# agnusmaximus/DistributedMNIST

Measured on AMD Instinct MI355X. Metric: images/sec (whole node), MNIST CNN sync-SGD, higher is better.
Workload: dtype bf16; 1 GPU; model=lenet, global_batch=1024, parallelism=dp1, mode=full_sync, mode_requested=full_sync, grad_dtype=fp32

## Files before the change

csrc/bindings.cpp:

```cpp

#include <torch/extension.h>
#include <ATen/hip/HIPContext.h>
#include <hip/hip_runtime.h>

#include <atomic>
#include <map>
#include <tuple>

#include "kernels.h"

namespace {

#define CHECK_BF16(t) TORCH_CHECK((t).scalar_type() == at::kBFloat16, #t " must be bf16")
#define CHECK_F32(t) TORCH_CHECK((t).scalar_type() == at::kFloat, #t " must be fp32")
#define CHECK_CONTIG(t) TORCH_CHECK((t).is_contiguous(), #t " must be contiguous")
#define CHECK_CUDA(t) TORCH_CHECK((t).is_cuda(), #t " must be on GPU")

const unsigned short* bf16_ptr(const torch::Tensor& t) {
  return reinterpret_cast<const unsigned short*>(t.data_ptr());
}
unsigned short* bf16_mut(torch::Tensor& t) {
  return reinterpret_cast<unsigned short*>(t.data_ptr());
}

// ... 693 lines not shown
      d[1].n = 32; d[1].stride = CONV1_DET_PLANE; d[1].P = blocks;
      nd = 2;
    }
    launch_plane_reduce(d, nd, s);
    return;
  }
  if (conv1_mfma_supported(H, W, 1, Cout) && conv1_mfma_enabled() &&
      reinterpret_cast<uintptr_t>(x.data_ptr()) % 8 == 0) {
    launch_conv1_mfma_dw(bf16_ptr(x), bf16_ptr(dyp), am.data_ptr<uint8_t>(),
                         dw_out.data_ptr<float>(),
                         db_out.defined() ? db_out.data_ptr<float>() : nullptr,
                         NB, cur_stream());
    return;
  }
  launch_conv1_dw_pooled(bf16_ptr(x), bf16_ptr(dyp),
                         am.data_ptr<uint8_t>(), dw_out.data_ptr<float>(),
                         db_out.defined() ? db_out.data_ptr<float>() : nullptr,
                         NB, H, W, Cout, cur_stream());
}

torch::Tensor conv_dx(torch::Tensor dact, torch::Tensor w, int64_t Cin) {
  CHECK_BF16(dact); CHECK_CONTIG(dact); CHECK_BF16(w); CHECK_CONTIG(w);
  return conv_dx_step(dact, w, (int)Cin, cur_stream());
}

static void check_pooled(const torch::Tensor& gp, const torch::Tensor& am) {
  CHECK_CUDA(gp); CHECK_BF16(gp); CHECK_CONTIG(gp);
  CHECK_CUDA(am); CHECK_CONTIG(am);
  TORCH_CHECK(am.scalar_type() == at::kByte, "am must be uint8");
  TORCH_CHECK(gp.dim() == 4 && gp.size(1) == 7 && gp.size(2) == 7 &&
                  gp.size(3) == 64,
              "pooled conv2 backward: gp is [NB][7][7][64]");
  TORCH_CHECK(am.numel() == gp.numel(), "am / gp shape mismatch");
  TORCH_CHECK(((uintptr_t)gp.data_ptr() & 15) == 0 &&
                  ((uintptr_t)am.data_ptr() & 7) == 0,
              "pooled conv2 backward: gp 16 B / am 8 B alignment");
}

torch::Tensor conv_dx_pooled(torch::Tensor gp, torch::Tensor am,
                             torch::Tensor w, int64_t Cin, int64_t force_db) {
  check_pooled(gp, am);
  CHECK_BF16(w); CHECK_CONTIG(w);
  TORCH_CHECK(Cin == 32 && w.numel() == 25 * 32 * 64,
              "conv_dx_pooled: LeNet conv2 shapes only");
  TORCH_CHECK(force_db >= 0 && force_db <= 2, "force_db is 0, 1 or 2");
  int NB = gp.size(0);
  auto dx = torch::empty({NB, 14, 14, 32}, gp.options());
  if (NB > 0)
    launch_conv_dx_slab_pooled(bf16_ptr(gp), am.data_ptr<uint8_t>(),
                               bf16_ptr(w), bf16_mut(dx), NB, (int)force_db,
                               cur_stream());
  return dx;
}

void conv_dw_pooled_into(torch::Tensor x, torch::Tensor gp, torch::Tensor am,
                         torch::Tensor dw_out) {
  check_pooled(gp, am);
  CHECK_CUDA(x); CHECK_BF16(x); CHECK_CONTIG(x);
  CHECK_F32(dw_out); CHECK_CONTIG(dw_out);
  TORCH_CHECK(x.dim() == 4 && x.size(0) == gp.size(0) && x.size(1) == 14 &&
                  x.size(2) == 14 && x.size(3) == 32,
              "conv_dw_pooled_into: x is [NB][14][14][32]");
  TORCH_CHECK(dw_out.numel() == 25 * 32 * 64, "conv_dw_pooled_into: dw size");
  TORCH_CHECK(((uintptr_t)x.data_ptr() & 15) == 0, "x 16 B alignment");
  if (det_on()) {
    int NB = x.size(0);
    if (NB <= 0) return;
    auto s = cur_stream();
    int groups = conv2_dw_groups(NB);
    float* planes = det_region(DET_CONV2_DW, x, CONV2_DET_PLANE, groups, s,
                               "conv_dw_pooled_into", "raise DMNIST_DW2_G");
    launch_conv2_dw_slab_pooled_det(bf16_ptr(x), bf16_ptr(gp),
                                    am.data_ptr<uint8_t>(), planes, NB, s);
    reduce_planes(planes, dw_out.data_ptr<float>(), CONV2_DET_PLANE,
                  CONV2_DET_PLANE, groups, s);
    return;
  }
  launch_conv2_dw_slab_pooled(bf16_ptr(x), bf16_ptr(gp),
                              am.data_ptr<uint8_t>(),
                              dw_out.data_ptr<float>(), (int)x.size(0),
                              cur_stream());
}

std::vector<torch::Tensor> softmax_xent_fwd(torch::Tensor logits,
                                            torch::Tensor labels,
                                            c10::optional<torch::Tensor> db_out,
                                            double inv_n) {
  CHECK_CUDA(logits); CHECK_BF16(logits); CHECK_CONTIG(logits);
  TORCH_CHECK(labels.scalar_type() == at::kLong, "labels must be int64");
  CHECK_CONTIG(labels);
  int B = logits.size(0), C = logits.size(1);
  TORCH_CHECK(C <= 16, "softmax_xent kernel supports C<=16");
  TORCH_CHECK(B <= 256 * SOFTMAX_MAX_BLOCKS, "softmax_xent: batch too large");
  auto dl = torch::empty_like(logits);
  auto out = torch::empty({2}, logits.options().dtype(at::kFloat));
  static auto* ws = new WorkspaceSlots(64);
  float* part = device_workspace(
      *ws, logits, 2 * SOFTMAX_MAX_BLOCKS + 1, at::kFloat, cur_stream(),
      "softmax_xent",
      "softmax_xent_fwd: first call on a device allocates its "
      "workspace and must run outside graph capture").data_ptr<float>();
  unsigned* ticket = reinterpret_cast<unsigned*>(part + 2 * SOFTMAX_MAX_BLOCKS);
  float* dbp = nullptr;
  if (db_out.has_value() && db_out->defined())
    dbp = db_out->data_ptr<float>();
  if (det_on() && dbp && B > 0) {
    auto s = cur_stream();
    int blocks = softmax_xent_blocks(B);
    float* planes = det_region(DET_SOFTMAX_DB, logits, C, blocks, s,
                               "softmax_xent_fwd", "lower the batch size");
    launch_softmax_xent_det(bf16_ptr(logits), labels.data_ptr<long>(),
                            bf16_mut(dl), out.data_ptr<float>(), B, C, planes,
                            (float)inv_n, part, ticket, s);
    reduce_planes(planes, dbp, C, C, blocks, s);
  } else {
    launch_softmax_xent(bf16_ptr(logits), labels.data_ptr<long>(),
                        bf16_mut(dl), out.data_ptr<float>(), B, C, dbp,
                        (float)inv_n, part, ticket, cur_stream());
  }
  auto loss = out.select(0, 0);
  auto correct = out.select(0, 1);
  return {loss, correct, dl};
}

static float* ema_ptr(const c10::optional<torch::Tensor>& ema,
                      const torch::Tensor& master, double ema_decay) {
  if (!ema.has_value() || !ema->defined()) return nullptr;
  CHECK_CUDA((*ema)); CHECK_F32((*ema)); CHECK_CONTIG((*ema));
  TORCH_CHECK(ema->numel() >= master.numel(),
              "sgd_step: ema is shorter than master");
  TORCH_CHECK(reinterpret_cast<uintptr_t>(ema->data_ptr()) % 16 == 0,
              "sgd_step: ema must be 16-byte aligned");
  TORCH_CHECK(ema_decay >= 0.0 && ema_decay < 1.0,
              "sgd_step: ema_decay must lie in [0, 1)");
  return ema->data_ptr<float>();
}

static float* momentum_ptr(const c10::optional<torch::Tensor>& momentum) {
  if (!momentum.has_value() || !momentum->defined()) return nullptr;
  CHECK_F32((*momentum)); CHECK_CONTIG((*momentum));
  return momentum->data_ptr<float>();
}

void sgd_step(torch::Tensor master, torch::Tensor grad, torch::Tensor shadow,
              bool has_shadow, double lr, double scale, double dc_keep,
              int64_t seed, int64_t offset,
              c10::optional<torch::Tensor> momentum, double mu,
              c10::optional<torch::Tensor> ema, double ema_decay) {
  CHECK_CUDA(master); CHECK_F32(master); CHECK_CONTIG(master);
  CHECK_F32(grad); CHECK_CONTIG(grad);
  float* mom = momentum_ptr(momentum);
  float* emap = ema_ptr(ema, master, ema_decay);
  launch_sgd_step(master.data_ptr<float>(), grad.data_ptr<float>(),
                  has_shadow ? bf16_mut(shadow) : nullptr,
                  has_shadow ? 1 : 0, master.numel(),
                  (float)(lr * scale), (float)dc_keep, (uint64_t)seed,
                  (uint64_t)offset, mom, (float)mu, emap, (float)ema_decay,
                  cur_stream());
}

void sgd_step_dev(torch::Tensor master, torch::Tensor grad,
                  torch::Tensor shadow, bool has_shadow,
                  torch::Tensor lr_scale_dev, double dc_keep, int64_t seed,
                  torch::Tensor offset_dev,
                  c10::optional<torch::Tensor> momentum, double mu,
                  bool zero_grad, c10::optional<torch::Tensor> ema,
                  double ema_decay) {
  CHECK_CUDA(master); CHECK_F32(master); CHECK_CONTIG(master);
  CHECK_F32(grad); CHECK_CONTIG(grad);
  CHECK_F32(lr_scale_dev);
  float* mom = momentum_ptr(momentum);
  launch_sgd_step_dev(master.data_ptr<float>(), grad.data_ptr<float>(),
                      has_shadow ? bf16_mut(shadow) : nullptr,
                      has_shadow ? 1 : 0, master.numel(),
                      lr_scale_dev.data_ptr<float>(), (float)dc_keep,
                      (uint64_t)seed, offset_dev.data_ptr<long>(),
                      mom, (float)mu, zero_grad ? 1 : 0,
                      ema_ptr(ema, master, ema_decay), (float)ema_decay,
                      cur_stream());
}

void ema_publish(torch::Tensor ema, torch::Tensor shadow,
                 std::vector<int64_t> offsets, std::vector<int64_t> rows,
                 std::vector<int64_t> cols, std::vector<torch::Tensor> dsts) {
  CHECK_CUDA(ema); CHECK_F32(ema); CHECK_CONTIG(ema);
  CHECK_CUDA(shadow); CHECK_BF16(shadow); CHECK_CONTIG(shadow);
  TORCH_CHECK(shadow.numel() == ema.numel(), "ema_publish: shadow size");
  TORCH_CHECK(reinterpret_cast<uintptr_t>(ema.data_ptr()) % 16 == 0 &&
              reinterpret_cast<uintptr_t>(shadow.data_ptr()) % 8 == 0,
              "ema_publish: ema must be 16-byte and shadow 8-byte aligned");
  size_t nt = dsts.size();
  TORCH_CHECK(nt <= 4 && offsets.size() == nt && rows.size() == nt &&
              cols.size() == nt, "ema_publish: up to 4 transposed tensors");
  EmaTransposeDesc d[4];
  for (size_t i = 0; i < nt; ++i) {
    CHECK_CUDA(dsts[i]); CHECK_BF16(dsts[i]); CHECK_CONTIG(dsts[i]);
    TORCH_CHECK(rows[i] > 0 && cols[i] > 0 && offsets[i] >= 0 &&
                rows[i] * cols[i] <= ema.numel() - offsets[i],
                "ema_publish: slice ", i, " lies outside the buffer");
    TORCH_CHECK(dsts[i].numel() == rows[i] * cols[i],
                "ema_publish: transposed copy ", i, " has the wrong size");
    d[i] = {(long)offsets[i], bf16_mut(dsts[i]), (int)rows[i], (int)cols[i]};
  }
  launch_ema_publish(ema.data_ptr<float>(), bf16_mut(shadow), ema.numel(), d,
                     (int)nt, cur_stream());
// ... 222 lines not shown
  hipGetDevice(&dev);
  std::vector<torch::Tensor> r;
  for (auto& kv : det_regions())
    if (std::get<0>(kv.first) == dev) r.push_back(kv.second);
  return r;
}

}

PYBIND11_MODULE(TORCH_EXTENSION_NAME, m) {
  m.def("set_deterministic", [](bool on) { g_deterministic.store(on); },
        "deterministic mode: gradient ops store per-block planes and reduce "
        "them in a fixed order; uncovered routes raise", py::arg("on"));
  m.def("get_deterministic", [] { return det_on(); });
  m.def("det_workspace", &det_workspace,
        "plane workspace tensors currently allocated on the current device");
  m.def("plane_reduce", &plane_reduce,
        "out[i] += ((p_0[i] + p_1[i]) + ...) + p_{P-1}[i] (fp32, index order)",
        py::arg("planes"), py::arg("out"));
  m.def("linear_act_fwd", &linear_act_fwd, "fused linear+bias+relu+dropout",
        py::arg("x"), py::arg("w"), py::arg("b"), py::arg("relu"),
        py::arg("p_keep"), py::arg("seed"), py::arg("offset"),
        py::arg("wT") = c10::nullopt);
  m.def("transpose_bf16", &transpose_bf16, "bf16 2-D transpose (wT refresh)");
  m.def("transpose_bf16_batch_adv", &transpose_bf16_batch_adv,
        "batched transposes + fused device step/LR advance (graph tail)");
  m.def("transpose_bf16_batch", &transpose_bf16_batch,
        "up to 4 transposes in one launch");
  m.def("mask_db", &mask_db, "relu/dropout grad mask + bias-grad column sums");
  m.def("linear_dw_into", &linear_dw_into, "dW = x^T dyeff into bucket view");
  m.def("linear_dx", &linear_dx, "dx = dyeff @ W^T");
  m.def("linear_dx_mask", &linear_dx_mask,
        "dx GEMM with fused relu/dropout mask + bias-grad column sums",
        py::arg("dyeff"), py::arg("w"), py::arg("actm"), py::arg("db_out"),
        py::arg("p_keep"));
  m.def("linear_dx_unpool", &linear_dx_unpool,
        "dx GEMM fused with maxpool2x2 backward scatter + conv db",
        py::arg("dyeff"), py::arg("w"), py::arg("amax"),
        py::arg("db_out"), py::arg("Ho"), py::arg("Wo"), py::arg("C"));
  m.def("linear_dx_pooled", &linear_dx_pooled,
        "dx GEMM masked by the pool argmax byte + conv db: pooled gradient",
        py::arg("dyeff"), py::arg("w"), py::arg("amax"),
        py::arg("db_out"), py::arg("Ho"), py::arg("Wo"), py::arg("C"),
        py::arg("tile") = 0);
  m.def("linear_dx_pooled_tile", [](int64_t B, int64_t K) {
          return (int64_t)(cdiv((int)B, 128) * cdiv((int)K, 128) >=
                                   POOLED_DX_BIG_TILES ? 128 : 64);
        }, "tile linear_dx_pooled picks for dyeff[B,*], w[K,*]");
  m.def("conv_dx_pooled", &conv_dx_pooled,
        "conv2 dX from the pooled gradient + pool argmax bytes",
        py::arg("gp"), py::arg("am"), py::arg("w"), py::arg("Cin"),
        py::arg("force_db") = 0);
  m.def("conv_dw_pooled_into", &conv_dw_pooled_into,
        "conv2 dW from the pooled gradient + pool argmax bytes, into bucket",
        py::arg("x"), py::arg("gp"), py::arg("am"), py::arg("dw_out"));
  m.def("linear_dw_plan", [](int64_t K, int64_t N, int64_t B) {
    DwPlan pl = linear_dw_plan((int)K, (int)N, (int)B);
    return std::make_tuple(pl.tbm, pl.bn, pl.splitk);
  }, "(tbm, bn, splitk) the fc dW launcher picks for x[B,K], dyeff[B,N]");
  m.def("pool_scatter", &pool_scatter, "maxpool bwd scatter + conv db");
  m.def("conv_dw_into", &conv_dw_into, "conv dW into bucket view");
  m.def("conv1_dw_pooled", &conv1_dw_pooled,
        "conv1 dW+db from the pooled gradient (pool bwd fused, no dact1)",
        py::arg("x"), py::arg("dyp"), py::arg("am"),
        py::arg("dw_out"), py::arg("db_out"));
  m.def("conv1_dw_group", [](int64_t NB) {
          return (int64_t)conv1_mfma_dw_group((int)NB);
        }, "images per block the MFMA conv1 dW launcher picks for batch NB");
  m.def("conv2_dw_group", [](int64_t NB) {
          return (int64_t)conv2_dw_group((int)NB);
        }, "images per block the slab conv2 dW launcher picks for batch NB");
  m.def("conv_dx", &conv_dx, "conv dX");
  m.def("linear_act_bwd", &linear_act_bwd, "linear backward (dx, dw, db)");
  m.def("linear_act_bwd_into", &linear_act_bwd_into,
        "linear backward accumulating dw/db into bucket views");
  m.def("conv_pool_fwd", &conv_pool_fwd, "fused conv5x5+bias+relu+maxpool",
        py::arg("x"), py::arg("w"), py::arg("b"), py::arg("wT") = c10::nullopt);
  m.def("conv_pool_bwd", &conv_pool_bwd, "conv+pool backward (dx, dw, db)");
  m.def("conv_pool_bwd_into", &conv_pool_bwd_into,
        "conv backward accumulating dw/db into bucket views");
  m.def("softmax_xent_fwd", &softmax_xent_fwd, "fused softmax-CE (+grad, +optional fc2 db, +optional acc-mean scale)",
        py::arg("logits"), py::arg("labels"),
        py::arg("db_out") = c10::nullopt, py::arg("inv_n") = 1.0);
  m.def("sgd_step", &sgd_step, "fused flat SGD(+momentum) apply",
        py::arg("master"), py::arg("grad"), py::arg("shadow"),
        py::arg("has_shadow"), py::arg("lr"), py::arg("scale"),
        py::arg("dc_keep"), py::arg("seed"), py::arg("offset"),
        py::arg("momentum") = c10::nullopt, py::arg("mu") = 0.0,
        py::arg("ema") = c10::nullopt, py::arg("ema_decay") = 0.0);
  m.def("ema_publish", &ema_publish,
        "flat fp32 parameters -> flat bf16 shadow + transposed bf16 copies "
        "of the [rows][cols] slices at `offsets`, one launch",
        py::arg("ema"), py::arg("shadow"), py::arg("offsets"),
        py::arg("rows"), py::arg("cols"), py::arg("dsts"));
  m.def("sgd_step_dev", &sgd_step_dev,
        "SGD apply with device-side lr/offset (hipGraph-capturable); "
        "zero_grad clears the bucket in the same pass",
        py::arg("master"), py::arg("grad"), py::arg("shadow"),
        py::arg("has_shadow"), py::arg("lr_scale_dev"), py::arg("dc_keep"),
        py::arg("seed"), py::arg("offset_dev"),
        py::arg("momentum") = c10::nullopt, py::arg("mu") = 0.0,
        py::arg("zero_grad") = false,
        py::arg("ema") = c10::nullopt, py::arg("ema_decay") = 0.0);
  m.def("step_advance", &step_advance,
        "device-side staircase LR + step increment (inside the graph)");
  m.def("grad_mask", &grad_mask,
        "per-rank pre-aggregation drop-connect mask (in-place, philox; "
        "reference distributed_train.py:194-203)",
        py::arg("g"), py::arg("keep"), py::arg("seed"), py::arg("step"),
        py::arg("rank"), py::arg("base") = 0,
        py::arg("step_dev") = c10::nullopt);
  m.def("batch_gather", &batch_gather,
        "gather one training batch from the device-resident uint8 set "
        "(Feistel epoch permutation keyed on seed + step; LUT-normalised "
        "to bf16) into x [B,28,28,1] bf16 / y [B] int64",
        py::arg("img_u8"), py::arg("lab_u8"), py::arg("lut"), py::arg("x"),
        py::arg("y"), py::arg("seed"), py::arg("step"),
        py::arg("step_dev") = c10::nullopt);
  m.def("batch_gather_aug", &batch_gather_aug,
        "batch_gather with on-device affine augmentation: image j is warped "
        "(integer bilinear, zero background) by row aug_indices(seed, step, "
        "j) of the int32 [T,6] Q16 inverse-affine table before the LUT",
        py::arg("img_u8"), py::arg("lab_u8"), py::arg("lut"),
        py::arg("table"), py::arg("x"), py::arg("y"), py::arg("seed"),
        py::arg("step"), py::arg("step_dev") = c10::nullopt);
  m.def("range_gather", &range_gather,
        "sequential chunk [start, start+B) of the device-resident uint8 set "
        "(LUT-normalised to bf16) into x [B,28,28,1] bf16 / y [B] int64; "
        "rows past N are zero-filled with label -1",
        py::arg("img_u8"), py::arg("lab_u8"), py::arg("lut"), py::arg("x"),
        py::arg("y"), py::arg("start"),
        py::arg("start_dev") = c10::nullopt);
  m.def("softmax_eval", &softmax_eval,
        "evaluation statistics accumulated across launches: loss_sum[1] "
        "fp32, counts[2 + C*C] int32 (live, correct, confusion), optional "
        "pred[B] uint8 and cursor_dev += B; rows with a label outside "
        "[0, C) contribute to nothing",
        py::arg("logits"), py::arg("labels"), py::arg("loss_sum"),
        py::arg("counts"), py::arg("pred") = c10::nullopt,
        py::arg("cursor_dev") = c10::nullopt);
  m.def("linear_act_fwd_dev", &linear_act_fwd_dev,
        "linear fwd with device-side dropout offset",
        py::arg("x"), py::arg("w"), py::arg("b"), py::arg("relu"),
        py::arg("p_keep"), py::arg("seed"), py::arg("offset_dev"),
        py::arg("wT") = c10::nullopt);
}
```

csrc/build.py:

```python
#!/usr/bin/env python3

import os
import subprocess
import sys
import sysconfig

ROOT = os.path.dirname(os.path.abspath(__file__))


def main():
    import torch
    import torch.utils.cpp_extension as ce

    torch_inc = ce.include_paths()
    torch_lib = ce.library_paths()[0]
    py_inc = sysconfig.get_paths()["include"]
    hipcc = os.environ.get("HIPCC", "/opt/rocm/bin/hipcc")
    abi = int(torch.compiled_with_cxx11_abi())

    srcs = [os.path.join(ROOT, f) for f in
            ("gemm_tile.hip", "conv_slab.hip", "dw_tr.hip", "ops_misc.hip", "conv1_mfma.hip",
             "data_gather.hip", "conv2_dw_slab.hip", "eval_ops.hip",
             "det_reduce.hip",
             "bindings.cpp")]
    out = os.path.join(ROOT, "_dmnist_hip.so")

    cmd = [hipcc, "--offload-arch=gfx950", "-O3", "-std=c++17", "-fPIC",
           "-shared", "-x", "hip"] + srcs + [
        "-o", out,
        f"-D_GLIBCXX_USE_CXX11_ABI={abi}",
        "-DTORCH_EXTENSION_NAME=_dmnist_hip",
        "-DTORCH_API_INCLUDE_EXTENSION_H",
        "-DUSE_ROCM=1", "-D__HIP_PLATFORM_AMD__=1",
        "-DHIP_ENABLE_WARP_SYNC_BUILTINS=1",
        "-fno-gpu-rdc",
        "-Wno-deprecated-declarations",
    ]
    cmd += [f"-I{p}" for p in torch_inc + [py_inc, ROOT]]
    cmd += [f"-L{torch_lib}", "-ltorch", "-ltorch_cpu", "-ltorch_hip",
            "-lc10", "-lc10_hip", "-ltorch_python",
            "-L/opt/rocm/lib", "-lamdhip64",
            f"-Wl,-rpath,{torch_lib}", "-Wl,-rpath,/opt/rocm/lib"]
    print("[build]", " ".join(cmd), flush=True)
    subprocess.run(cmd, check=True)
    print(f"[build] wrote {out}")


if __name__ == "__main__":
    main()
```

csrc/kernels.h:

```cpp
#pragma once
#include <hip/hip_runtime.h>
#include <stdint.h>

struct GemmParams {
  const unsigned short* A;
  const unsigned short* B;
  const float* bias;
  void* C;
  uint8_t* amax;
  int M, N, K;
  int lda, ldb, ldc;
  int splitk;
  int CB, CH, CW, CHo, CWo, Cin, Cout;
  float p_keep;
  uint64_t seed, offset;
  const long* offset_dev;
  float* db;
  const unsigned short* actm;
  int unpool_lines;
  unsigned* tickets;
  unsigned short* Y;
  int relu;
  float* det_planes;
  long det_stride;
};

void gemm_fwd_bias_128(const GemmParams&, hipStream_t);
void gemm_fwd_bias_64(const GemmParams&, hipStream_t);
void gemm_fwd_relu_128(const GemmParams&, hipStream_t);
void gemm_fwd_relu_64(const GemmParams&, hipStream_t);
void gemm_fwd_drop_128(const GemmParams&, hipStream_t);
void gemm_fwd_drop_64(const GemmParams&, hipStream_t);
void gemm_dx_128(const GemmParams&, hipStream_t);
void gemm_dx_64(const GemmParams&, hipStream_t);
void gemm_dx_unpool_128(const GemmParams&, hipStream_t);
void gemm_dx_unpool_64(const GemmParams&, hipStream_t);
void gemm_dx_poolmask_128(const GemmParams&, hipStream_t);
void gemm_dx_poolmask_64(const GemmParams&, hipStream_t);
void gemm_dx_mask_128(const GemmParams&, hipStream_t);
void gemm_dx_mask_64(const GemmParams&, hipStream_t);
void gemm_dw_128(const GemmParams&, hipStream_t);
void gemm_dw_64(const GemmParams&, hipStream_t);
void conv_fwd_pool(const GemmParams&, hipStream_t);
void conv1_fwd_pool(const GemmParams&, hipStream_t);
void conv_dx_gemm(const GemmParams&, hipStream_t);
void conv_dw_gemm(const GemmParams&, hipStream_t);
void conv_dw_tr(const GemmParams&, hipStream_t);
void gemm_dw_tr(const GemmParams&, int tbm, int bn, bool single_writer,
                hipStream_t);
void gemm_dw_tr_det(const GemmParams&, int tbm, int bn, hipStream_t);

void launch_relu_drop_bwd(const unsigned short* dy, const unsigned short* y,
                          unsigned short* dyeff, float* db, int B, int N,
                          float inv_keep, int apply_mask, hipStream_t);
void launch_pool_bwd_scatter(const unsigned short* dy, const unsigned short* y,
                             const uint8_t* amax, unsigned short* dact,
                             float* db, int Mpool, int C, int H, int W, int Wo,
                             hipStream_t);
#define SOFTMAX_MAX_BLOCKS 4096
void launch_softmax_xent(const unsigned short* logits, const long* labels,
                         unsigned short* dlogits, float* out, int B, int C,
                         float* db, float inv_n, float* part,
                         unsigned* ticket, hipStream_t);
int softmax_xent_blocks(int B);
void launch_softmax_xent_det(const unsigned short* logits, const long* labels,
                             unsigned short* dlogits, float* out, int B, int C,
                             float* dbplanes, float inv_n, float* part,
                             unsigned* ticket, hipStream_t);
void launch_sgd_step(float* master, float* grad, unsigned short* shadow,
                     int has_shadow, long n, float lr_scale, float dc_keep,
                     uint64_t seed, uint64_t offset, float* momentum, float mu,
                     float* ema, float ema_decay, hipStream_t);
void launch_sgd_step_dev(float* master, float* grad,
                         unsigned short* shadow, int has_shadow, long n,
                         const float* lr_scale_dev, float dc_keep,
                         uint64_t seed, const long* offset_dev,
                         float* momentum, float mu, int zero_grad,
                         float* ema, float ema_decay, hipStream_t);
struct EmaTransposeDesc {
  long offset;
  unsigned short* dst;
  int R, C;
};
struct EmaPublishArgs {
  const float* src;
  unsigned short* shadow;
  long n;
  EmaTransposeDesc d[4];
  int tile0[4];
  int nt, flat_blocks;
};
void launch_ema_publish(const float* src, unsigned short* shadow, long n,
                        const EmaTransposeDesc* descs, int nt, hipStream_t);
void launch_conv1_dw_pooled(const unsigned short* x, const unsigned short* dyp,
                            const uint8_t* am, float* dw, float* db, int NB,
                            int H, int W, int Cout, hipStream_t s);
void launch_grad_mask(float* g, long n, long base, float keep, uint64_t seed,
                      uint64_t step, uint64_t rank, const long* step_dev,
                      hipStream_t s);
void launch_step_advance(long* step_dev, float* lr_scale_dev, float lr0,
                         float decay, int decay_steps, float inv_contrib,
                         hipStream_t);
void launch_batch_gather(const uint8_t* img, const uint8_t* lab,
                         const unsigned short* lut, unsigned short* x,
                         long* y, uint32_t N, uint32_t B, uint64_t seed,
                         uint64_t step, const long* step_dev, hipStream_t);
void launch_batch_gather_aug(const uint8_t* img, const uint8_t* lab,
                             const unsigned short* lut, const int* table,
                             uint32_t T, unsigned short* x, long* y,
                             uint32_t N, uint32_t B, uint64_t seed,
                             uint64_t step, const long* step_dev,
                             hipStream_t);
void launch_range_gather(const uint8_t* img, const uint8_t* lab,
                         const unsigned short* lut, unsigned short* x,
                         long* y, uint32_t N, uint32_t B, uint64_t start,
                         const long* start_dev, hipStream_t);
void launch_softmax_eval(const unsigned short* logits, const long* labels,
                         float* loss_sum, int* counts, uint8_t* pred,
                         long* cursor_dev, int B, int C, float* part,
                         unsigned* ticket, hipStream_t);
void launch_transpose_bf16(const unsigned short* src, unsigned short* dst,
                           int R, int C, hipStream_t);
struct TransposeDesc {
  const unsigned short* src;
  unsigned short* dst;
  int R, C;
};
struct TransposeBatchArgs {
  TransposeDesc d[4];
  int tile0[4];
  int n, total;
  int do_advance;
  long* step_dev;
  float* lr_scale_dev;
  float lr0, decay, inv_contrib;
  int decay_steps;
};
void launch_transpose_bf16_batch(const TransposeDesc* descs, int n,
                                 hipStream_t);
void launch_transpose_bf16_batch_adv(const TransposeDesc* descs, int n,
                                     long* step_dev, float* lr_scale_dev,
                                     float lr0, float decay, int decay_steps,
                                     float inv_contrib, hipStream_t);
void launch_conv1_direct_fwd(const unsigned short* x, const unsigned short* w,
                             const float* bias, unsigned short* y,
                             uint8_t* amax, int NB, int H, int W, int Cout,
                             hipStream_t);
void gemm_dx_poolmask_128_det(const GemmParams&, hipStream_t);
void gemm_dx_poolmask_64_det(const GemmParams&, hipStream_t);
void gemm_dx_mask_128_det(const GemmParams&, hipStream_t);
void gemm_dx_mask_64_det(const GemmParams&, hipStream_t);
// ... 87 lines not shown
```

distributedmnist_amd/engine/fused_step.py:

```python

from __future__ import annotations

import torch
import torch.distributed as dist

from .. import _C


class FusedLeNetStep:
    def __init__(self, trainer):
        t = trainer
        m = t.model
        from ..models import LeNet5
        assert isinstance(m, LeNet5), "fused step is LeNet-specific"
        assert t.compute_dtype == torch.bfloat16 and t.device.type == "cuda"
        assert m.shadows and m.shadows_T, "fused step needs bf16 shadows"
        self.t = t
        self.ext = _C.ext()
        import os as _os
        if _os.environ.get("DMNIST_OVERLAP"):
            self.overlap_level = int(_os.environ["DMNIST_OVERLAP"])
        elif _os.environ.get("DMNIST_TWO_STREAM"):
            self.overlap_level = 2
        elif _os.environ.get("DMNIST_SINGLE_STREAM"):
            self.overlap_level = 0
        else:
            self.overlap_level = 0 if t.flags.batch_size < 4096 else 2
        self.single_stream = self.overlap_level == 0
        self.pool2_fused = _os.environ.get("DMNIST_POOL2_FUSED", "1") != "0"
        self.side = None if self.single_stream else torch.cuda.Stream()
        self.p_keep = 0.5
        self.seed = t.flags.seed
        fp = t.fp
        fc0 = fp.offsets[fp.names.index("fc1_w")]
        self.fc_offset = fc0
        self.conv_slice = fp.flat_grad[:fc0]
        self.fc_slice = fp.flat_grad[fc0:]
        self.overlap_allreduce = t.world > 1 and dist.is_initialized()

    def _fork(self, a, b):
        if not self.single_stream:
            a.wait_stream(b)

    def __call__(self, x, labels, step_dev):
        reduce_grads = self.overlap_allreduce
        loss, acc, conv_in, self._keep = self._fc_part(x, labels, step_dev,
                                                       reduce_grads)
        self._conv_part(*conv_in)
        if reduce_grads:
            self.t.engine.wire_allreduce(self.conv_slice, start=0)
        return loss, acc

    def stage_fc(self, x, labels, step_dev):
        loss, acc, self._stash, self._keep = self._fc_part(
            x, labels, step_dev, False)
        s0, s1 = self._streams()
        s0.wait_stream(s1)
        return loss, acc

    def stage_conv(self):
        self._conv_part(*self._stash)
        self._keep2 = self._stash

    def _gv(self, name):
        return getattr(self.t.model, name).grad

    def _streams(self):
        s0 = torch.cuda.current_stream()
        return s0, (s0 if self.single_stream else self.side)

    def _fc_part(self, x, labels, step_dev, reduce_fc):
        ext, gv = self.ext, self._gv
        m = self.t.model
        sh, shT = m.shadows, m.shadows_T
        B = x.shape[0]
        s0, s1 = self._streams()

        y1, am1 = ext.conv_pool_fwd(x, sh["conv1_w"], m.conv1_b, None)
        y2, am2 = ext.conv_pool_fwd(y1, sh["conv2_w"], m.conv2_b,
                                    shT["conv2_w"])
        h2 = y2.view(B, 7 * 7 * 64)
        a1 = ext.linear_act_fwd_dev(h2, sh["fc1_w"], m.fc1_b, True,
                                    self.p_keep, self.seed, step_dev,
                                    shT["fc1_w"])
        logits = ext.linear_act_fwd(a1, sh["fc2_w"], m.fc2_b, False, 1.0,
                                    0, 0, shT["fc2_w"])
        loss, acc, dl = ext.softmax_xent_fwd(logits, labels,
                                             db_out=gv("fc2_b"),
                                             inv_n=1.0 / B)

        self._fork(s1, s0)
        with torch.cuda.stream(s1):
            ext.linear_dw_into(a1, dl, gv("fc2_w"))
        dyeff1 = ext.linear_dx_mask(dl, sh["fc2_w"], a1, gv("fc1_b"),
                                    self.p_keep)
        self._fork(s1, s0)
        with torch.cuda.stream(s1):
            ext.linear_dw_into(h2, dyeff1, gv("fc1_w"))
            if reduce_fc:
                self.t.engine.wire_allreduce(self.fc_slice,
                                             start=self.fc_offset)
        g2 = self._fc1_dx(dyeff1, am2)
        keep = (a1, h2, dyeff1, dl, y1, g2, am2)
        return loss, acc, (x, y1, am1, g2, am2), keep

    def _conv_part(self, x, y1, am1, g2, am2):
        s0, s1 = self._streams()
        sW = s1 if self.overlap_level >= 2 else s0
        if sW is not s0:
            self._fork(sW, s0)
        with torch.cuda.stream(sW):
            self._conv2_dw(y1, g2, am2)
        dxc = self._conv2_dx(g2, am2)
        self.ext.conv1_dw_pooled(x, dxc, am1, self._gv("conv1_w"),
                                 self._gv("conv1_b"))
        self._fork(s0, s1)

    def _fc1_dx(self, dyeff1, am2):
        m = self.t.model
        f = (self.ext.linear_dx_pooled if self.pool2_fused
             else self.ext.linear_dx_unpool)
        return f(dyeff1, m.shadows["fc1_w"], am2, m.conv2_b.grad, 7, 7, 64)

    def _conv2_dw(self, y1, g2, am2):
        dw = self.t.model.conv2_w.grad
        if self.pool2_fused:
            self.ext.conv_dw_pooled_into(y1, g2, am2, dw)
        else:
            self.ext.conv_dw_into(y1, g2, dw)

    def _conv2_dx(self, g2, am2):
        w = self.t.model.shadows["conv2_w"]
        if self.pool2_fused:
            return self.ext.conv_dx_pooled(g2, am2, w, 32)
        return self.ext.conv_dx(g2, w, 32)
```

distributedmnist_amd/ops/cpu_ref.py:

```python

from __future__ import annotations

import torch
import torch.nn.functional as F



def conv_pool_fwd(x, w, b):
    N, H, W, Cin = x.shape
    Cout = w.shape[3]
    xc = x.permute(0, 3, 1, 2)
    wc = w.permute(3, 2, 0, 1)
    conv = F.conv2d(xc.float(), wc.float(), b.float(), padding=2)
    act = F.relu(conv)
    pooled, idx = F.max_pool2d(act, 2, 2, return_indices=True)
    Ho, Wo = pooled.shape[2], pooled.shape[3]
    ar = torch.arange(Ho, device=x.device).view(1, 1, Ho, 1)
    ac = torch.arange(Wo, device=x.device).view(1, 1, 1, Wo)
    r = idx // W - ar * 2
    c = idx % W - ac * 2
    amax = (r * 2 + c).to(torch.uint8)
    amax = torch.where(pooled > 0, amax,
                       torch.tensor(7, dtype=torch.uint8))
    y = pooled.permute(0, 2, 3, 1).contiguous()
    amax = amax.permute(0, 2, 3, 1).contiguous()
    return y, amax


def conv_pool_bwd(dy, x, w, y, amax):
    N, Ho, Wo, Cout = dy.shape
    H, W = Ho * 2, Wo * 2
    Cin = x.shape[3]
    g = (dy * (y > 0)).permute(0, 3, 1, 2).float()
    am = amax.permute(0, 3, 1, 2).long().clamp(max=3)
    dact = x.new_zeros((N, Cout, H, W), dtype=torch.float32)
    ar = torch.arange(Ho, device=x.device).view(1, 1, Ho, 1)
    ac = torch.arange(Wo, device=x.device).view(1, 1, 1, Wo)
    rows = ar * 2 + am // 2
    cols = ac * 2 + am % 2
    flat = (rows * W + cols)
    dact.view(N, Cout, H * W).scatter_(2, flat.view(N, Cout, -1),
                                       g.view(N, Cout, -1))
    xc = x.permute(0, 3, 1, 2).float()
    wc = w.permute(3, 2, 0, 1).float()
    dxc = torch.nn.grad.conv2d_input(xc.shape, wc, dact, padding=2)
    dwc = torch.nn.grad.conv2d_weight(xc, wc.shape, dact, padding=2)
    db = dact.sum(dim=(0, 2, 3))
    dx = dxc.permute(0, 2, 3, 1).contiguous().to(x.dtype)
    dw = dwc.permute(2, 3, 1, 0).contiguous()
    return dx, dw, db



def linear_fwd(x, w, b, relu: bool = False):
    y = x.float() @ w.float() + b.float()
    if relu:
        y = F.relu(y)
    return y.to(x.dtype)


def linear_bwd(dy, x, w, y=None, relu: bool = False):
    dyf = dy.float()
    if relu:
        dyf = dyf * (y > 0)
    dx = (dyf @ w.float().t()).to(x.dtype)
    dw = x.float().t() @ dyf
    db = dyf.sum(dim=0)
    return dx, dw, db


def dropout_fwd(x, p_drop: float, gen: torch.Generator | None = None):
    keep = 1.0 - p_drop
    mask = (torch.rand(x.shape, device="cpu", dtype=torch.float32,
                       generator=gen) < keep).to(x.device)
    y = x * mask.to(x.dtype) / keep
    return y.to(x.dtype), mask


def dropout_bwd(dy, mask, p_drop: float):
    keep = 1.0 - p_drop
    return (dy * mask.to(dy.dtype) / keep).to(dy.dtype)



def softmax_xent_fwd(logits, labels):
    lf = logits.float()
    m = lf.max(dim=1, keepdim=True).values
    z = lf - m
    ez = z.exp()
    se = ez.sum(dim=1, keepdim=True)
    logp = z - se.log()
    B = logits.shape[0]
    loss = -logp.gather(1, labels.view(-1, 1)).mean()
    p = ez / se
    dl = p
    dl.scatter_add_(1, labels.view(-1, 1), torch.full((B, 1), -1.0, device=logits.device))
    dl = (dl / B).to(logits.dtype)
    correct = (lf.argmax(dim=1) == labels).float().sum()
    return loss, correct, dl



def sgd_step(master, grad, lr: float, grad_scale: float = 1.0,
             drop_connect_keep: float | None = None,
             gen: torch.Generator | None = None, shadow=None,
             momentum=None, mu: float = 0.0, ema=None,
             ema_decay: float = 0.0, offset: int = 0):
    g = grad.float() * grad_scale
    if drop_connect_keep is not None:
        mask = (torch.rand(g.shape, device=g.device, dtype=torch.float32,
                           generator=gen) < drop_connect_keep).float()
        g = g * mask
    if momentum is not None:
        momentum.mul_(mu).add_(g)
        g = momentum
    master.add_(g, alpha=-lr)
    if ema is not None:
        ema.sub_((ema - master) * ema_weight(ema_decay, offset))
    if shadow is not None:
        shadow.copy_(master.to(shadow.dtype))
    return master


def ema_weight(ema_decay: float, offset: int) -> float:
    if not 0.0 <= ema_decay < 1.0:
        raise ValueError(f"ema_decay must lie in [0, 1), got {ema_decay}")
    import numpy as np
    k = np.float32(int(offset) + 1)
    d = min(np.float32(ema_decay),
            (np.float32(1) + k) / (np.float32(10) + k))
    return float(np.float32(1) - d)



_M32 = 0xFFFFFFFF


def _mix32(x):
    x = x ^ (x >> 16)
    x = (x * 0x85EBCA6B) & _M32
    x = x ^ (x >> 13)
    x = (x * 0xC2B2AE35) & _M32
    return x ^ (x >> 16)


def feistel_perm(n: int, seed: int, epoch: int, p):
    import numpy as np
    p = np.asarray(p, dtype=np.int64)
    if p.size and not (0 <= p.min() and p.max() < n):
        raise ValueError(f"positions must lie in [0, {n})")
    if epoch == 0:
        return p.copy()
    seed &= 0xFFFFFFFFFFFFFFFF
    base = _mix32((seed & _M32) ^ _mix32(((seed >> 32) + 0x9E3779B9) & _M32))
    keys = [_mix32((base + (epoch & _M32) * 0x9E3779B1 + r) & _M32)
            for r in range(4)]
    bits = max(2, (n - 1).bit_length())
    bits += bits & 1
    h = np.uint64(bits // 2)
    mask = np.uint64((1 << (bits // 2)) - 1)
    m32 = np.uint64(_M32)

    def enc(v):
        L, R = v >> h, v & mask
        for k in keys:
            f = _mix32((R * np.uint64(0x9E3779B1) + np.uint64(k)) & m32)
            L, R = R, L ^ (f & mask)
        return (L << h) | R

    v = enc(p.astype(np.uint64))
    out = v >= np.uint64(n)
    while out.any():
        v[out] = enc(v[out])
        out = v >= np.uint64(n)
    return v.astype(np.int64)


def batch_indices(n: int, batch_size: int, seed: int, step: int):
    import numpy as np
    if not 1 <= batch_size <= n:
        raise ValueError(f"batch size {batch_size} must be in [1, N={n}]")
    if step < 0:
        raise ValueError("step must be >= 0")
    spe = n // batch_size
# ... 147 lines not shown
```

Baseline: 3.877 million images/sec.

## Fuse fc2 forward, softmax-xent, fc2 dW and masked dX into one kernel

Adds a single HIP kernel that computes the fc2 logits with MFMA, the softmax cross-entropy loss and gradient, the fc2 bias and weight gradients, and the masked fc1 dX plus fc1 bias gradient, all while keeping tiles in shared memory. The training step now calls it in place of four launches and a stream fork, which is meant to cut launch overhead and global-memory round trips for the logits and dlogits. In exchange, fc2 dW and the biases are accumulated with per-block atomics, which adds contention and makes the sums order-dependent. The fused path needs C=10 and K=512 and falls back to the separate steps otherwise.

Measured after the change: 4.108 million images/sec, median of 6. 6.0% higher.

```diff
diff --git a/csrc/bindings.cpp b/csrc/bindings.cpp
--- a/csrc/bindings.cpp
+++ b/csrc/bindings.cpp
@@ -799,6 +799,14 @@
                               cur_stream());
 }
 
+float* softmax_workspace(const torch::Tensor& like, hipStream_t s) {
+  static auto* ws = new WorkspaceSlots(64);
+  return device_workspace(
+      *ws, like, 2 * SOFTMAX_MAX_BLOCKS + 1, at::kFloat, s, "softmax_xent",
+      "softmax_xent_fwd / fc2_head: first call on a device allocates its "
+      "workspace and must run outside graph capture").data_ptr<float>();
+}
+
 std::vector<torch::Tensor> softmax_xent_fwd(torch::Tensor logits,
                                             torch::Tensor labels,
                                             c10::optional<torch::Tensor> db_out,
@@ -811,12 +819,7 @@
   TORCH_CHECK(B <= 256 * SOFTMAX_MAX_BLOCKS, "softmax_xent: batch too large");
   auto dl = torch::empty_like(logits);
   auto out = torch::empty({2}, logits.options().dtype(at::kFloat));
-  static auto* ws = new WorkspaceSlots(64);
-  float* part = device_workspace(
-      *ws, logits, 2 * SOFTMAX_MAX_BLOCKS + 1, at::kFloat, cur_stream(),
-      "softmax_xent",
-      "softmax_xent_fwd: first call on a device allocates its "
-      "workspace and must run outside graph capture").data_ptr<float>();
+  float* part = softmax_workspace(logits, cur_stream());
   unsigned* ticket = reinterpret_cast<unsigned*>(part + 2 * SOFTMAX_MAX_BLOCKS);
   float* dbp = nullptr;
   if (db_out.has_value() && db_out->defined())
@@ -838,6 +841,74 @@
   auto loss = out.select(0, 0);
   auto correct = out.select(0, 1);
   return {loss, correct, dl};
+}
+
+int fc2_head_rows(int B) {
+  if (const char* e = getenv("DMNIST_FC2_R")) {
+    int r = atoi(e);
+    if (r == 16 || r == 32 || r == 64) return r;
+  }
+  return B < 160 ? 32 : 64;
+}
+
+std::vector<torch::Tensor> fc2_head(torch::Tensor a1, torch::Tensor w2,
+                                    torch::Tensor w2T, torch::Tensor b2,
+                                    torch::Tensor labels,
+                                    torch::Tensor dw2_out,
+                                    torch::Tensor db2_out,
+                                    torch::Tensor db1_out, double p_keep,
+                                    double inv_n) {
+  CHECK_CUDA(a1); CHECK_BF16(a1); CHECK_CONTIG(a1);
+  CHECK_BF16(w2); CHECK_CONTIG(w2);
+  CHECK_BF16(w2T); CHECK_CONTIG(w2T);
+  CHECK_F32(b2); CHECK_CONTIG(b2);
+  TORCH_CHECK(labels.scalar_type() == at::kLong, "labels must be int64");
+  CHECK_CONTIG(labels);
+  CHECK_F32(dw2_out); CHECK_CONTIG(dw2_out);
+  CHECK_F32(db2_out); CHECK_CONTIG(db2_out);
+  CHECK_F32(db1_out); CHECK_CONTIG(db1_out);
+  TORCH_CHECK(a1.dim() == 2 && w2.dim() == 2 && w2T.dim() == 2,
+              "fc2_head: a1, w2 and w2T are 2-D");
+  const int64_t B = a1.size(0), K = a1.size(1), C = w2.size(1);
+  TORCH_CHECK(w2.size(0) == K, "fc2_head: w2 is [K][C]");
+  TORCH_CHECK(w2T.size(0) == C && w2T.size(1) == K, "fc2_head: w2T is [C][K]");
+  TORCH_CHECK(b2.numel() == C && db2_out.numel() == C,
+              "fc2_head: b2 and db2_out hold C values");
+  TORCH_CHECK(dw2_out.numel() == K * C, "fc2_head: dw2_out holds K*C values");
+  TORCH_CHECK(db1_out.numel() == K, "fc2_head: db1_out holds K values");
+  TORCH_CHECK(labels.numel() == B, "fc2_head: one label per row");
+  TORCH_CHECK(p_keep > 0.0 && p_keep <= 1.0, "fc2_head: p_keep in (0, 1]");
+  TORCH_CHECK(B <= 256 * SOFTMAX_MAX_BLOCKS, "fc2_head: batch too large");
+  auto s = cur_stream();
+
+  const char* fe = getenv("DMNIST_FC2_FUSED");
+  const int R = fc2_head_rows((int)B);
+  const bool fused =
+      !(fe && atoi(fe) == 0) && !det_on() && B > 0 && C == 10 &&
+      K == FC2_HEAD_K &&
+      fc2_head_blocks((int)B, R) <= SOFTMAX_MAX_BLOCKS &&
+      ((uintptr_t)a1.data_ptr() & 15) == 0 &&
+      ((uintptr_t)w2T.data_ptr() & 15) == 0;
+  if (!fused) {
+    auto logits = linear_act_fwd_impl(a1, w2, b2, false, 1.0, 0, 0, nullptr,
+                                      w2T);
+    auto sm = softmax_xent_fwd(logits, labels, db2_out, inv_n);
+    linear_dw_step(a1, sm[2], dw2_out.data_ptr(), s);
+    auto dyeff1 = linear_dx_mask(sm[2], w2, a1, db1_out, p_keep);
+    return {sm[0], sm[1], dyeff1};
+  }
+  auto dyeff1 = torch::empty_like(a1);
+  TORCH_CHECK(((uintptr_t)dyeff1.data_ptr() & 15) == 0,
+              "fc2_head: dyeff1 must be 16-byte aligned");
+  auto out = torch::empty({2}, a1.options().dtype(at::kFloat));
+  float* part = softmax_workspace(a1, s);
+  unsigned* ticket = reinterpret_cast<unsigned*>(part + 2 * SOFTMAX_MAX_BLOCKS);
+  launch_fc2_head(R, bf16_ptr(a1), bf16_ptr(w2T), b2.data_ptr<float>(),
+                  labels.data_ptr<long>(), bf16_mut(dyeff1),
+                  dw2_out.data_ptr<float>(), db2_out.data_ptr<float>(),
+                  db1_out.data_ptr<float>(), out.data_ptr<float>(), (int)B,
+                  (float)(1.0 / p_keep), (float)inv_n, part, ticket, s);
+  return {out.select(0, 0), out.select(0, 1), dyeff1};
 }
 
 static float* ema_ptr(const c10::optional<torch::Tensor>& ema,
@@ -1226,6 +1297,15 @@
   m.def("softmax_xent_fwd", &softmax_xent_fwd, "fused softmax-CE (+grad, +optional fc2 db, +optional acc-mean scale)",
         py::arg("logits"), py::arg("labels"),
         py::arg("db_out") = c10::nullopt, py::arg("inv_n") = 1.0);
+  m.def("fc2_head", &fc2_head,
+        "fc2 forward + softmax-xent (+db2) + fc2 dW + fc2 dX with the fc1 "
+        "mask (+db1): one launch, or the four separate steps; returns "
+        "(loss, acc, dyeff1)",
+        py::arg("a1"), py::arg("w2"), py::arg("w2T"), py::arg("b2"),
+        py::arg("labels"), py::arg("dw2_out"), py::arg("db2_out"),
+        py::arg("db1_out"), py::arg("p_keep"), py::arg("inv_n") = 1.0);
+  m.def("fc2_head_rows", [](int64_t B) { return fc2_head_rows((int)B); },
+        "rows per block the fused fc2 head picks at batch size B");
   m.def("sgd_step", &sgd_step, "fused flat SGD(+momentum) apply",
         py::arg("master"), py::arg("grad"), py::arg("shadow"),
         py::arg("has_shadow"), py::arg("lr"), py::arg("scale"),
diff --git a/csrc/build.py b/csrc/build.py
--- a/csrc/build.py
+++ b/csrc/build.py
@@ -21,7 +21,7 @@
     srcs = [os.path.join(ROOT, f) for f in
             ("gemm_tile.hip", "conv_slab.hip", "dw_tr.hip", "ops_misc.hip", "conv1_mfma.hip",
              "data_gather.hip", "conv2_dw_slab.hip", "eval_ops.hip",
-             "det_reduce.hip",
+             "det_reduce.hip", "fc2_head.hip",
              "bindings.cpp")]
     out = os.path.join(ROOT, "_dmnist_hip.so")
 
diff --git a/csrc/fc2_head.hip b/csrc/fc2_head.hip
--- /dev/null
+++ b/csrc/fc2_head.hip
@@ -0,0 +1,303 @@
+
+#include "common.h"
+#include "kernels.h"
+
+#define FC2H_PITCH (FC2_HEAD_K + 16)
+#define FC2H_C 10
+#define FC2H_WPG 4
+
+DEV float row_sum16(float x) {
+#define FC2H_ROR(n)                                                         \
+  x += __builtin_bit_cast(float, __builtin_amdgcn_update_dpp(               \
+           0, __builtin_bit_cast(int, x), 0x120 + (n), 0xf, 0xf, false))
+  FC2H_ROR(8);
+  FC2H_ROR(4);
+  FC2H_ROR(2);
+  FC2H_ROR(1);
+#undef FC2H_ROR
+  return x;
+}
+
+template <int R>
+__global__ __launch_bounds__(R * 4 * FC2H_WPG)
+void fc2_head_kernel(const ushort_t* a1, const ushort_t* w2T, const float* b2,
+                     const long* labels, ushort_t* dyeff, float* dw2,
+                     float* db2, float* db1, float* out, int B,
+                     float inv_keep, float inv_n, float* part,
+                     unsigned* ticket) {
+  constexpr int K = FC2_HEAD_K;
+  constexpr int C = FC2H_C;
+  constexpr int WPG = FC2H_WPG;
+  constexpr int NG = R / 16;
+  constexpr int NW = NG * WPG;
+  constexpr int NT = NW * 64;
+  static_assert(K == 512, "a row is 64 chunks of 16 B: one per lane");
+  static_assert(NT <= 1024 && 1024 % NT == 0 && (K / 16) % NW == 0, "split");
+  __shared__ __attribute__((aligned(16))) ushort_t a_s[R][FC2H_PITCH];
+  __shared__ __attribute__((aligned(16))) ushort_t wT_s[16][FC2H_PITCH];
+  __shared__ __attribute__((aligned(16))) ushort_t wp_s[K][16];
+  __shared__ __attribute__((aligned(16))) ushort_t lg_s[R][16];
+  __shared__ __attribute__((aligned(16))) ushort_t dl_s[R][16];
+  __shared__ float db2_s[NG][16];
+  __shared__ float lc_s[NG][2];
+  __shared__ __attribute__((aligned(16))) float db1_s[NG][K];
+
+  const int tid = threadIdx.x;
+  const int lane = tid & 63, wv = tid >> 6;
+  const int grp = wv / WPG, prt = wv % WPG;
+  const int r = lane & 15, h = lane >> 4;
+  const int row0 = blockIdx.x * R;
+  const int grow = grp * 16;
+  const bool head = prt == 0;
+
+  const int brow = row0 + grow + r;
+  const bool live = head && h == 0 && brow < B;
+  const int lab = live ? (int)labels[brow] : 0;
+  const float bias = (head && r < C) ? b2[r] : 0.f;
+  {
+    constexpr int AI = 16 / WPG;
+    uint4 v[AI];
+#pragma unroll
+    for (int i = 0; i < AI; ++i) {
+      int gr = row0 + grow + prt + i * WPG;
+      v[i] = uint4{0u, 0u, 0u, 0u};
+      if (gr < B)
+        v[i] = *reinterpret_cast<const uint4*>(a1 + (size_t)gr * K + lane * 8);
+    }
+    constexpr int WI = 16 * 64 / NT;
+    uint4 w[WI];
+#pragma unroll
+    for (int it = 0; it < WI; ++it) {
+      int i = tid + it * NT;
+      int rr = i >> 6, ch = i & 63;
+      w[it] = uint4{0u, 0u, 0u, 0u};
+      if (rr < C)
+        w[it] = *reinterpret_cast<const uint4*>(w2T + (size_t)rr * K + ch * 8);
+    }
+#pragma unroll
+    for (int i = 0; i < AI; ++i)
+      *reinterpret_cast<uint4*>(&a_s[grow + prt + i * WPG][lane * 8]) = v[i];
+#pragma unroll
+    for (int it = 0; it < WI; ++it) {
+      int i = tid + it * NT;
+      int rr = i >> 6, ch = i & 63;
+      *reinterpret_cast<uint4*>(&wT_s[rr][ch * 8]) = w[it];
+    }
+  }
+  __syncthreads();
+
+  if (!head) {
+    constexpr int BT = NG * (WPG - 1) * 64;
+    const int bt = (grp * (WPG - 1) + prt - 1) * 64 + lane;
+#pragma unroll
+    for (int n = bt; n < K; n += BT) {
+      union { ushort_t u[16]; uint4 v[2]; } row;
+#pragma unroll
+      for (int c = 0; c < 16; ++c) row.u[c] = c < C ? wT_s[c][n] : (ushort_t)0;
+      *reinterpret_cast<uint4*>(&wp_s[n][0]) = row.v[0];
+      *reinterpret_cast<uint4*>(&wp_s[n][8]) = row.v[1];
+    }
+  } else {
+    f32x4 acc = {0.f, 0.f, 0.f, 0.f};
+    const ushort_t* ap = &a_s[grow + r][8 * h];
+    const ushort_t* bp = &wT_s[r][8 * h];
+#pragma unroll
+    for (int kk = 0; kk < K; kk += 32) {
+      short8 a = *reinterpret_cast<const short8*>(ap + kk);
+      short8 b = *reinterpret_cast<const short8*>(bp + kk);
+      acc = __builtin_amdgcn_mfma_f32_16x16x32_bf16(a, b, acc, 0, 0, 0);
+    }
+#pragma unroll
+    for (int q = 0; q < 4; ++q)
+      lg_s[grow + 4 * h + q][r] = r < C ? f2bf(acc[q] + bias) : (ushort_t)0;
+    __builtin_amdgcn_fence(__ATOMIC_RELEASE, "workgroup");
+    __builtin_amdgcn_wave_barrier();
+    __builtin_amdgcn_fence(__ATOMIC_ACQUIRE, "workgroup");
+
+    float d[C];
+    float loss = 0.f, correct = 0.f;
+    {
+      float v[C];
+      float mx = -1e30f;
+      int arg = 0;
+#pragma unroll
+      for (int c = 0; c < C; ++c) {
+        v[c] = bf2f(lg_s[grow + r][c]);
+        if (v[c] > mx) { mx = v[c]; arg = c; }
+      }
+      float se = 0.f;
+#pragma unroll
+      for (int c = 0; c < C; ++c) {
+        v[c] = __expf(v[c] - mx);
+        se += v[c];
+      }
+      float inv_se = 1.f / se;
+      float invB = 1.f / (float)B;
+      float vlab = 0.f;
+      union { ushort_t u[16]; uint4 q[2]; } rowo;
+#pragma unroll
+      for (int c = 0; c < 16; ++c) rowo.u[c] = 0;
+#pragma unroll
+      for (int c = 0; c < C; ++c) {
+        float pp = v[c] * inv_se;
+        d[c] = live ? (pp - (c == lab ? 1.f : 0.f)) * invB : 0.f;
+        rowo.u[c] = f2bf(d[c]);
+        if (c == lab) vlab = v[c];
+      }
+      if (h == 0) {
+        *reinterpret_cast<uint4*>(&dl_s[grow + r][0]) = rowo.q[0];
+        *reinterpret_cast<uint4*>(&dl_s[grow + r][8]) = rowo.q[1];
+      }
+      if (live) {
+        loss = -(__logf(vlab * inv_se)) * invB;
+        correct = (arg == lab) ? 1.f : 0.f;
+      }
+    }
+    float ls = row_sum16(loss), cs = row_sum16(correct * inv_n);
+    if (lane == 0) {
+      lc_s[grp][0] = ls;
+      lc_s[grp][1] = cs;
+    }
+#pragma unroll
+    for (int c = 0; c < C; ++c) {
+      float dsum = row_sum16(d[c]);
+      if (lane == 0) db2_s[grp][c] = dsum;
+    }
+  }
+  __syncthreads();
+
+  if (wv == NW - 1 && lane < C) {
+    float v = db2_s[0][lane];
+    for (int g = 1; g < NG; ++g) v += db2_s[g][lane];
+    if (v != 0.f) atomicAdd(&db2[lane], v);
+  }
+  if (wv == NW - 1 && lane == 0) {
+    const unsigned nblk = gridDim.x;
+    float r0 = 0.f, r1 = 0.f;
+    for (int g = 0; g < NG; ++g) {
+      r0 += lc_s[g][0];
+      r1 += lc_s[g][1];
+    }
+    if (nblk == 1) {
+      out[0] = r0;
+      out[1] = r1;
+    } else {
+      __hip_atomic_store(&part[2 * blockIdx.x], r0, __ATOMIC_RELAXED,
+                         __HIP_MEMORY_SCOPE_AGENT);
+      __hip_atomic_store(&part[2 * blockIdx.x + 1], r1, __ATOMIC_RELAXED,
+                         __HIP_MEMORY_SCOPE_AGENT);
+      __threadfence();
+      if (atomicAdd(ticket, 1u) == nblk - 1) {
+        __threadfence();
+        float s0 = 0.f, s1 = 0.f;
+        for (unsigned i = 0; i < nblk; ++i) {
+          s0 += __hip_atomic_load(&part[2 * i], __ATOMIC_RELAXED,
+                                  __HIP_MEMORY_SCOPE_AGENT);
+          s1 += __hip_atomic_load(&part[2 * i + 1], __ATOMIC_RELAXED,
+                                  __HIP_MEMORY_SCOPE_AGENT);
+        }
+        out[0] = s0;
+        out[1] = s1;
+        __hip_atomic_store(ticket, 0u, __ATOMIC_RELAXED,
+                           __HIP_MEMORY_SCOPE_AGENT);
+      }
+    }
+  }
+
+  {
+    constexpr int KS = R >= 32 ? R / 32 : 1;
+    short8 bfr[KS];
+#pragma unroll
+    for (int ks = 0; ks < KS; ++ks)
+#pragma unroll
+      for (int j = 0; j < 8; ++j) {
+        int row = ks * 32 + 8 * h + j;
+        bfr[ks][j] = row < R ? (short)dl_s[row < R ? row : 0][r] : (short)0;
+      }
+#pragma unroll
+    for (int i = 0; i < (K >> 4) / NW; ++i) {
+      const int t = wv + i * NW;
+      f32x4 acc = {0.f, 0.f, 0.f, 0.f};
+#pragma unroll
+      for (int ks = 0; ks < KS; ++ks) {
+        short8 afr;
+#pragma unroll
+        for (int j = 0; j < 8; ++j) {
+          int row = ks * 32 + 8 * h + j;
+          afr[j] = row < R ? (short)a_s[row < R ? row : 0][t * 16 + r]
+                           : (short)0;
+        }
+        acc = __builtin_amdgcn_mfma_f32_16x16x32_bf16(afr, bfr[ks], acc, 0, 0, 0);
+      }
+      if (r < C) {
+#pragma unroll
+        for (int q = 0; q < 4; ++q)
+          atomicAdd(&dw2[(size_t)(t * 16 + 4 * h + q) * C + r], acc[q]);
+      }
+    }
+  }
+  __syncthreads();
+
+  {
+    short8 bfr = {0, 0, 0, 0, 0, 0, 0, 0};
+    if (h < 2) bfr = *reinterpret_cast<const short8*>(&dl_s[grow + r][8 * h]);
+    constexpr int TW = (K >> 4) / WPG;
+#pragma unroll
+    for (int i = 0; i < TW; ++i) {
+      const int t = prt * TW + i;
+      short8 afr = {0, 0, 0, 0, 0, 0, 0, 0};
+      if (h < 2) afr = *reinterpret_cast<const short8*>(&wp_s[t * 16 + r][8 * h]);
+      f32x4 acc = {0.f, 0.f, 0.f, 0.f};
+      acc = __builtin_amdgcn_mfma_f32_16x16x32_bf16(afr, bfr, acc, 0, 0, 0);
+      const int n = t * 16 + 4 * h;
+      union { ushort_t u[4]; uint2 v; } e;
+      e.v = *reinterpret_cast<const uint2*>(&a_s[grow + r][n]);
+      float s[4];
+#pragma unroll
+      for (int q = 0; q < 4; ++q) {
+        float v = (bf2f(e.u[q]) > 0.f) ? acc[q] * inv_keep : 0.f;
+        e.u[q] = f2bf(v);
+        s[q] = row_sum16(v);
+      }
+      *reinterpret_cast<uint2*>(&a_s[grow + r][n]) = e.v;
+      if (r == 0)
+        *reinterpret_cast<float4*>(&db1_s[grp][n]) =
+            float4{s[0], s[1], s[2], s[3]};
+    }
+  }
+  __syncthreads();
+#pragma unroll
+  for (int i = 0; i < 16 / WPG; ++i) {
+    int rr = prt + i * WPG;
+    int gr = row0 + grow + rr;
+    if (gr < B)
+      *reinterpret_cast<uint4*>(dyeff + (size_t)gr * K + lane * 8) =
+          *reinterpret_cast<const uint4*>(&a_s[grow + rr][lane * 8]);
+  }
+#pragma unroll
+  for (int n = tid; n < K; n += NT) {
+    float s = db1_s[0][n];
+#pragma unroll
+    for (int g = 1; g < NG; ++g) s += db1_s[g][n];
+    atomicAdd(&db1[n], s);
+  }
+}
+
+int fc2_head_blocks(int B, int R) { return (B + R - 1) / R; }
+
+void launch_fc2_head(int R, const unsigned short* a1,
+                     const unsigned short* w2T, const float* b2,
+                     const long* labels, unsigned short* dyeff, float* dw2,
+                     float* db2, float* db1, float* out, int B,
+                     float inv_keep, float inv_n, float* part,
+                     unsigned* ticket, hipStream_t s) {
+  dim3 grid(fc2_head_blocks(B, R));
+#define FC2H_LAUNCH(RR)                                                      \
+  hipLaunchKernelGGL((fc2_head_kernel<RR>), grid, dim3(RR * 4 * FC2H_WPG),   \
+                     0, s, a1, w2T, b2, labels, dyeff, dw2, db2, db1, out,   \
+                     B, inv_keep, inv_n, part, ticket)
+  if (R == 16) FC2H_LAUNCH(16);
+  else if (R == 32) FC2H_LAUNCH(32);
+  else FC2H_LAUNCH(64);
+#undef FC2H_LAUNCH
+}
diff --git a/csrc/kernels.h b/csrc/kernels.h
--- a/csrc/kernels.h
+++ b/csrc/kernels.h
@@ -67,6 +67,14 @@
                              unsigned short* dlogits, float* out, int B, int C,
                              float* dbplanes, float inv_n, float* part,
                              unsigned* ticket, hipStream_t);
+#define FC2_HEAD_K 512
+int fc2_head_blocks(int B, int R);
+void launch_fc2_head(int R, const unsigned short* a1,
+                     const unsigned short* w2T, const float* b2,
+                     const long* labels, unsigned short* dyeff, float* dw2,
+                     float* db2, float* db1, float* out, int B,
+                     float inv_keep, float inv_n, float* part,
+                     unsigned* ticket, hipStream_t);
 void launch_sgd_step(float* master, float* grad, unsigned short* shadow,
                      int has_shadow, long n, float lr_scale, float dc_keep,
                      uint64_t seed, uint64_t offset, float* momentum, float mu,
diff --git a/distributedmnist_amd/engine/fused_step.py b/distributedmnist_amd/engine/fused_step.py
--- a/distributedmnist_amd/engine/fused_step.py
+++ b/distributedmnist_amd/engine/fused_step.py
@@ -83,17 +83,11 @@
         a1 = ext.linear_act_fwd_dev(h2, sh["fc1_w"], m.fc1_b, True,
                                     self.p_keep, self.seed, step_dev,
                                     shT["fc1_w"])
-        logits = ext.linear_act_fwd(a1, sh["fc2_w"], m.fc2_b, False, 1.0,
-                                    0, 0, shT["fc2_w"])
-        loss, acc, dl = ext.softmax_xent_fwd(logits, labels,
-                                             db_out=gv("fc2_b"),
-                                             inv_n=1.0 / B)
+        loss, acc, dyeff1 = ext.fc2_head(a1, sh["fc2_w"], shT["fc2_w"],
+                                         m.fc2_b, labels, gv("fc2_w"),
+                                         gv("fc2_b"), gv("fc1_b"),
+                                         self.p_keep, 1.0 / B)
 
-        self._fork(s1, s0)
-        with torch.cuda.stream(s1):
-            ext.linear_dw_into(a1, dl, gv("fc2_w"))
-        dyeff1 = ext.linear_dx_mask(dl, sh["fc2_w"], a1, gv("fc1_b"),
-                                    self.p_keep)
         self._fork(s1, s0)
         with torch.cuda.stream(s1):
             ext.linear_dw_into(h2, dyeff1, gv("fc1_w"))
@@ -101,7 +95,7 @@
                 self.t.engine.wire_allreduce(self.fc_slice,
                                              start=self.fc_offset)
         g2 = self._fc1_dx(dyeff1, am2)
-        keep = (a1, h2, dyeff1, dl, y1, g2, am2)
+        keep = (a1, h2, dyeff1, y1, g2, am2)
         return loss, acc, (x, y1, am1, g2, am2), keep
 
     def _conv_part(self, x, y1, am1, g2, am2):
diff --git a/distributedmnist_amd/ops/cpu_ref.py b/distributedmnist_amd/ops/cpu_ref.py
--- a/distributedmnist_amd/ops/cpu_ref.py
+++ b/distributedmnist_amd/ops/cpu_ref.py
@@ -100,6 +100,25 @@
     return loss, correct, dl
 
 
+def fc2_head(a1, w2, b2, labels, p_keep: float):
+    B = a1.shape[0]
+    af, wf = a1.double(), w2.double()
+    logits = (af @ wf + b2.double()).to(a1.dtype).double()
+    z = logits - logits.max(dim=1, keepdim=True).values
+    ez = z.exp()
+    se = ez.sum(dim=1, keepdim=True)
+    onehot = torch.zeros_like(ez).scatter_(1, labels.view(-1, 1), 1.0)
+    loss = -((z - se.log()) * onehot).sum() / B
+    correct = (logits.argmax(dim=1) == labels).double().sum()
+    d = (ez / se - onehot) / B
+    db2 = d.sum(dim=0)
+    dl = d.to(a1.dtype).double()
+    dw2 = af.t() @ dl
+    g = (dl @ wf.t()) * (a1 > 0) / p_keep
+    db1 = g.sum(dim=0)
+    return loss, correct, g.to(a1.dtype), dw2, db1, db2
+
+
 
 def sgd_step(master, grad, lr: float, grad_scale: float = 1.0,
              drop_connect_keep: float | None = None,
```
